# danini/multi-h

Measured on AMD Instinct MI355X. Metric: scored homography hypotheses/sec (50k pts x 100k models), higher is better.
Workload: dtype f64

## Files before the change

### multi-h_amd/csrc/dlt4.hip

```cpp

#include "mh_kernels.hpp"
#include "mh_device.hpp"
#include "mh_sampler.hpp"

namespace mh {


__device__ __forceinline__ void rr_pair(int r, int slot, int& p, int& q)
{
    const int k = slot + 1;
    const int a = (r + k) % 9, b = (r + 9 - k) % 9;
    p = a < b ? a : b;
    q = a < b ? b : a;
}

constexpr int HPW = 16;
constexpr int WROWS = 17, WCOLS = 9;

__device__ __forceinline__ void wave_sync()
{
#ifdef MH_DLT_WAVE_FENCES
    __builtin_amdgcn_fence(__ATOMIC_RELEASE, "wavefront");
    __builtin_amdgcn_wave_barrier();
    __builtin_amdgcn_fence(__ATOMIC_ACQUIRE, "wavefront");
#else
    asm volatile("" ::: "memory");
    __builtin_amdgcn_wave_barrier();
    asm volatile("" ::: "memory");
#endif
}

__device__ __forceinline__ void null9_sweeps(double (*W)[HPW], int hs, int slot, bool live)
{
#define WE(r, c) W[(r) * WCOLS + (c)][hs]
    for (int sweep = 0; sweep < 30; ++sweep) {
        int rotated = 0;
        for (int r = 0; r < 9; ++r) {
            int p, q;
            rr_pair(r, slot, p, q);
            double alpha = 0.0, beta = 0.0, gamma = 0.0;
#pragma unroll
            for (int i = 0; i < 8; ++i) {
                const double wp = WE(i, p), wq = WE(i, q);
                alpha = alpha + wp * wp;
                beta = beta + wq * wq;
                gamma = gamma + wp * wq;
            }
            const bool rot = live && (gamma != 0.0) && (gamma * gamma > 1e-30 * (alpha * beta)) &&
                             (alpha >= 1e-28) && (beta >= 1e-28);
            if (rot) {
                ++rotated;
                const double zeta = (beta - alpha) / (2.0 * gamma);
                const double sg = (zeta >= 0.0) ? 1.0 : -1.0;
                const double t = sg / (fabs(zeta) + sqrt(1.0 + zeta * zeta));
                const double c = 1.0 / sqrt(1.0 + t * t);
                const double s = c * t;
#pragma unroll
                for (int i = 0; i < WROWS; ++i) {
                    const double wp = WE(i, p), wq = WE(i, q);
                    WE(i, p) = c * wp - s * wq;
                    WE(i, q) = s * wp + c * wq;
                }
            }
            wave_sync();
        }
        if (!__any(rotated)) break;
    }
#undef WE
}

__device__ __forceinline__ void null9_vector(double (*W)[HPW], int hs, double g[9])
{
#define WE(r, c) W[(r) * WCOLS + (c)][hs]
    int jm = 0;
    double best = 0.0;
    for (int j = 0; j < 9; ++j) {
        double a = 0.0;
        for (int i = 0; i < 8; ++i) a = a + WE(i, j) * WE(i, j);
        if (j == 0 || a < best) { best = a; jm = j; }
    }
    for (int j = 0; j < 9; ++j) g[j] = WE(8 + j, jm);
#undef WE
}

template <int SAMPLER, class... TABLE>
__global__ void __launch_bounds__(256) __attribute__((amdgpu_num_vgpr(72)))
k_dlt4_lds(const double* __restrict__ x1, const double* __restrict__ y1,
       const double* __restrict__ x2, const double* __restrict__ y2, int N,
       unsigned long long seed, long long first, int M, int* __restrict__ idx_out,
       double* __restrict__ H_out, TABLE... table)
{
    static_assert(sizeof...(TABLE) == dlt_sampler_args(SAMPLER), "the local sampler takes nbr, k, uniform_per_16; the segment sampler cluster_begin, trials, first");
    __builtin_amdgcn_s_setprio(3);
    __shared__ double sW[4][WROWS * WCOLS][HPW];
    const int lane = threadIdx.x & 63;
    const int wave = threadIdx.x >> 6;
    const int hs = lane & (HPW - 1);
    const int slot = lane >> 4;
    const int m = (blockIdx.x * 4 + wave) * HPW + hs;
    const bool live = m < M;
    double (*W)[HPW] = sW[wave];
#define WE(r, c) W[(r) * WCOLS + (c)][hs]

    int id[4] = { 0, 0, 0, 0 };
    double sx[4], sy[4], dx[4], dy[4];
    if (live) sample4_by(seed, (unsigned long long)(first + m), (unsigned int)N, id, table...);
#pragma unroll
    for (int k = 0; k < 4; ++k) {
        sx[k] = x1[id[k]]; sy[k] = y1[id[k]]; dx[k] = x2[id[k]]; dy[k] = y2[id[k]];
    }
    if (live && slot == 0 && idx_out) {
#pragma unroll
        for (int k = 0; k < 4; ++k) idx_out[4 * (size_t)m + k] = id[k];
    }
    double cx1 = ((sx[0] + sx[1]) + sx[2]) + sx[3], cy1 = ((sy[0] + sy[1]) + sy[2]) + sy[3];
    double cx2 = ((dx[0] + dx[1]) + dx[2]) + dx[3], cy2 = ((dy[0] + dy[1]) + dy[2]) + dy[3];
    cx1 = cx1 * 0.25; cy1 = cy1 * 0.25; cx2 = cx2 * 0.25; cy2 = cy2 * 0.25;
    double d1 = 0.0, d2 = 0.0;
#pragma unroll
    for (int k = 0; k < 4; ++k) {
        const double ax = sx[k] - cx1, ay = sy[k] - cy1, bx = dx[k] - cx2, by = dy[k] - cy2;
        d1 = d1 + sqrt(ax * ax + ay * ay);
        d2 = d2 + sqrt(bx * bx + by * by);
    }
    const double s1 = sqrt(2.0) / (d1 * 0.25), s2 = sqrt(2.0) / (d2 * 0.25);

    {
        double x = 0.0, y = 0.0, u = 0.0, v = 0.0;
#pragma unroll
        for (int k = 0; k < 4; ++k)
            if (k == slot) {
                x = (sx[k] - cx1) * s1; y = (sy[k] - cy1) * s1;
                u = (dx[k] - cx2) * s2; v = (dy[k] - cy2) * s2;
            }
        const int r0 = 2 * slot, r1 = 2 * slot + 1;
        WE(r0, 0) = -x; WE(r0, 1) = -y; WE(r0, 2) = -1.0; WE(r0, 3) = 0.0; WE(r0, 4) = 0.0;
        WE(r0, 5) = 0.0; WE(r0, 6) = u * x; WE(r0, 7) = u * y; WE(r0, 8) = u;
        WE(r1, 0) = 0.0; WE(r1, 1) = 0.0; WE(r1, 2) = 0.0; WE(r1, 3) = -x; WE(r1, 4) = -y;
        WE(r1, 5) = -1.0; WE(r1, 6) = v * x; WE(r1, 7) = v * y; WE(r1, 8) = v;
        if (slot < 3)
            for (int i = 3 * slot; i < 3 * slot + 3; ++i)
                for (int j = 0; j < 9; ++j) WE(8 + i, j) = (i == j) ? 1.0 : 0.0;
    }
    __syncthreads();

    null9_sweeps(W, hs, slot, live);

    if (live && slot == 0) {
        double g[9];
        null9_vector(W, hs, g);
        double A1[9];
#pragma unroll
        for (int r = 0; r < 3; ++r) {
            const double a = g[3 * r], b = g[3 * r + 1], c = g[3 * r + 2];
            A1[3 * r] = a * s1;
            A1[3 * r + 1] = b * s1;
            A1[3 * r + 2] = (c - (a * s1) * cx1) - (b * s1) * cy1;
        }
        const double is2 = 1.0 / s2;
        double Hh[9];
#pragma unroll
        for (int j = 0; j < 3; ++j) {
            Hh[j] = A1[j] * is2 + cx2 * A1[6 + j];
            Hh[3 + j] = A1[3 + j] * is2 + cy2 * A1[6 + j];
            Hh[6 + j] = A1[6 + j];
        }
        double fro = 0.0;
#pragma unroll
        for (int j = 0; j < 9; ++j) fro = fro + Hh[j] * Hh[j];
        double sc = 1.0 / sqrt(fro);
        if (Hh[8] < 0.0) sc = -sc;
        double* out = H_out + 9 * (size_t)m;
#pragma unroll
        for (int j = 0; j < 9; ++j) out[j] = Hh[j] * sc;
    }
#undef WE
}

struct Col { double v[WROWS]; };

template <int CTRL, int BANK_MASK>
__device__ __forceinline__ double dpp_merge(double old, double src)
{
    const int lo = __builtin_amdgcn_update_dpp(__double2loint(old), __double2loint(src), CTRL, 0xF, BANK_MASK, false);
    const int hi = __builtin_amdgcn_update_dpp(__double2hiint(old), __double2hiint(src), CTRL, 0xF, BANK_MASK, false);
    return __hiloint2double(hi, lo);
}

__device__ __forceinline__ void shift_columns(Col& a, Col& b, Col& c)
{
#pragma unroll
    for (int i = 0; i < WROWS; ++i) {
        c.v[i] = dpp_merge<0x114 , 0xE>(c.v[i], b.v[i]);
        b.v[i] = dpp_merge<0x104 , 0x7>(b.v[i], a.v[i]);
    }
}

__device__ __forceinline__ int rotate_pair(Col& P, Col& Q, bool swapped, bool live)
{
    double alpha = 0.0, beta = 0.0, gamma = 0.0;
#pragma unroll
    for (int i = 0; i < 8; ++i) {
        const double wp = P.v[i], wq = Q.v[i];
        alpha = alpha + wp * wp;
        beta = beta + wq * wq;
        gamma = gamma + wp * wq;
    }
    const bool rot = live && (gamma != 0.0) && (gamma * gamma > 1e-30 * (alpha * beta)) &&
                     (alpha >= 1e-28) && (beta >= 1e-28);
    if (rot) {
        const double zeta = (beta - alpha) / (2.0 * gamma);
        const bool pos = swapped ? (zeta > 0.0) : (zeta >= 0.0);
        const double sg = pos ? 1.0 : -1.0;
        const double t = sg / (fabs(zeta) + sqrt(1.0 + zeta * zeta));
        const double c = 1.0 / sqrt(1.0 + t * t);
        const double s = c * t;
#pragma unroll
        for (int i = 0; i < WROWS; ++i) {
            const double wp = P.v[i], wq = Q.v[i];
            P.v[i] = c * wp - s * wq;
            Q.v[i] = s * wp + c * wq;
        }
    }
    return rot ? 1 : 0;
}

__host__ __device__ constexpr unsigned swapped_rounds(int s)
{
    unsigned m = 0;
    for (int r = 0; r < 9; ++r) {
        const int k = s + 1, a = (r + k) % 9, b = (r + 9 - k) % 9;
        if (a > b) m |= 1u << r;
    }
    return m;
}

__device__ __forceinline__ void dlt_column(int c, const double* x, const double* y, const double* u, const double* v, Col& out)
{
#pragma unroll
    for (int k = 0; k < 4; ++k) {
        const double e0[9] = { -x[k], -y[k], -1.0, 0.0, 0.0, 0.0, u[k] * x[k], u[k] * y[k], u[k] };
        const double e1[9] = { 0.0, 0.0, 0.0, -x[k], -y[k], -1.0, v[k] * x[k], v[k] * y[k], v[k] };
        double r0 = e0[0], r1 = e1[0];
#pragma unroll
        for (int j = 1; j < 9; ++j) {
            r0 = (c == j) ? e0[j] : r0;
            r1 = (c == j) ? e1[j] : r1;
        }
        out.v[2 * k] = r0;
        out.v[2 * k + 1] = r1;
    }
#pragma unroll
    for (int i = 0; i < 9; ++i) out.v[8 + i] = (i == c) ? 1.0 : 0.0;
}

__device__ __forceinline__ double column_norm(const Col& a)
{
    double n = 0.0;
#pragma unroll
    for (int i = 0; i < 8; ++i) n = n + a.v[i] * a.v[i];
    return n;
}

template <int SAMPLER, class... TABLE>
__global__ void __launch_bounds__(256)
k_dlt4(const double* __restrict__ x1, const double* __restrict__ y1,
       const double* __restrict__ x2, const double* __restrict__ y2, int N,
       unsigned long long seed, long long first, int M, int* __restrict__ idx_out,
       double* __restrict__ H_out, TABLE... table)
{
    static_assert(sizeof...(TABLE) == dlt_sampler_args(SAMPLER), "the local sampler takes nbr, k, uniform_per_16; the segment sampler cluster_begin, trials, first");
    __builtin_amdgcn_s_setprio(3);
    __shared__ double sN[4][9][HPW];
    __shared__ double sK[4][6][HPW];
    const int lane = threadIdx.x & 63;
    const int wave = threadIdx.x >> 6;
    const int slot = (lane >> 2) & 3;
    const int hs = (lane >> 4) * 4 + (lane & 3);
    const int m = (blockIdx.x * 4 + wave) * HPW + hs;
    const bool live = m < M;

    Col A, B, C;
    {
        int id[4] = { 0, 0, 0, 0 };
        double sx[4], sy[4], dx[4], dy[4];
        if (live) sample4_by(seed, (unsigned long long)(first + m), (unsigned int)N, id, table...);
#pragma unroll
        for (int k = 0; k < 4; ++k) {
            sx[k] = x1[id[k]]; sy[k] = y1[id[k]]; dx[k] = x2[id[k]]; dy[k] = y2[id[k]];
        }
        if (live && slot == 0 && idx_out) {
#pragma unroll
            for (int k = 0; k < 4; ++k) idx_out[4 * (size_t)m + k] = id[k];
        }
        double cx1 = ((sx[0] + sx[1]) + sx[2]) + sx[3], cy1 = ((sy[0] + sy[1]) + sy[2]) + sy[3];
        double cx2 = ((dx[0] + dx[1]) + dx[2]) + dx[3], cy2 = ((dy[0] + dy[1]) + dy[2]) + dy[3];
        cx1 = cx1 * 0.25; cy1 = cy1 * 0.25; cx2 = cx2 * 0.25; cy2 = cy2 * 0.25;
        double d1 = 0.0, d2 = 0.0;
#pragma unroll
        for (int k = 0; k < 4; ++k) {
            const double ax = sx[k] - cx1, ay = sy[k] - cy1, bx = dx[k] - cx2, by = dy[k] - cy2;
            d1 = d1 + sqrt(ax * ax + ay * ay);
            d2 = d2 + sqrt(bx * bx + by * by);
        }
        const double s1 = sqrt(2.0) / (d1 * 0.25), s2 = sqrt(2.0) / (d2 * 0.25);
        if (slot == 0) {
            sK[wave][0][hs] = s1; sK[wave][1][hs] = s2; sK[wave][2][hs] = cx1;
            sK[wave][3][hs] = cy1; sK[wave][4][hs] = cx2; sK[wave][5][hs] = cy2;
        }
        double x[4], y[4], u[4], v[4];
#pragma unroll
        for (int k = 0; k < 4; ++k) {
            x[k] = (sx[k] - cx1) * s1; y[k] = (sy[k] - cy1) * s1;
            u[k] = (dx[k] - cx2) * s2; v[k] = (dy[k] - cy2) * s2;
        }
        dlt_column(slot + 1, x, y, u, v, A);
        dlt_column(8 - slot, x, y, u, v, B);
        dlt_column(0, x, y, u, v, C);
    }

    const unsigned sw = slot == 0 ? swapped_rounds(0) : slot == 1 ? swapped_rounds(1) : slot == 2 ? swapped_rounds(2) : swapped_rounds(3);
    for (int sweep = 0; sweep < 30; ++sweep) {
        unsigned long long rotated = 0;
#pragma unroll 1
        for (int r = 0; r < 9; r += 3) {
            rotated |= __ballot(rotate_pair(A, B, (sw >> r) & 1u, live));
            shift_columns(A, B, C);
            rotated |= __ballot(rotate_pair(B, C, (sw >> (r + 1)) & 1u, live));
            shift_columns(B, C, A);
            rotated |= __ballot(rotate_pair(C, A, (sw >> (r + 2)) & 1u, live));
            shift_columns(C, A, B);
        }
        if (rotated == 0) break;
    }

    sN[wave][slot + 1][hs] = column_norm(A);
    sN[wave][8 - slot][hs] = column_norm(B);
    if (slot == 0) sN[wave][0][hs] = column_norm(C);
    wave_sync();
    int jm = 0;
    {
        double best = 0.0;
        for (int j = 0; j < 9; ++j) {
            const double a = sN[wave][j][hs];
            if (j == 0 || a < best) { best = a; jm = j; }
        }
    }
    wave_sync();
    if (jm == slot + 1) {
#pragma unroll
        for (int j = 0; j < 9; ++j) sN[wave][j][hs] = A.v[8 + j];
    } else if (jm == 8 - slot) {
#pragma unroll
        for (int j = 0; j < 9; ++j) sN[wave][j][hs] = B.v[8 + j];
    } else if (jm == 0 && slot == 0) {
#pragma unroll
        for (int j = 0; j < 9; ++j) sN[wave][j][hs] = C.v[8 + j];
    }
    wave_sync();

    if (live && slot == 0) {
        double g[9];
#pragma unroll
        for (int j = 0; j < 9; ++j) g[j] = sN[wave][j][hs];
        const double s1 = sK[wave][0][hs], s2 = sK[wave][1][hs], cx1 = sK[wave][2][hs];
        const double cy1 = sK[wave][3][hs], cx2 = sK[wave][4][hs], cy2 = sK[wave][5][hs];
        double A1[9];
#pragma unroll
        for (int r = 0; r < 3; ++r) {
            const double a = g[3 * r], b = g[3 * r + 1], c = g[3 * r + 2];
            A1[3 * r] = a * s1;
            A1[3 * r + 1] = b * s1;
            A1[3 * r + 2] = (c - (a * s1) * cx1) - (b * s1) * cy1;
        }
        const double is2 = 1.0 / s2;
        double Hh[9];
#pragma unroll
        for (int j = 0; j < 3; ++j) {
            Hh[j] = A1[j] * is2 + cx2 * A1[6 + j];
            Hh[3 + j] = A1[3 + j] * is2 + cy2 * A1[6 + j];
            Hh[6 + j] = A1[6 + j];
        }
        double fro = 0.0;
#pragma unroll
        for (int j = 0; j < 9; ++j) fro = fro + Hh[j] * Hh[j];
        double sc = 1.0 / sqrt(fro);
        if (Hh[8] < 0.0) sc = -sc;
        double* out = H_out + 9 * (size_t)m;
#pragma unroll
        for (int j = 0; j < 9; ++j) out[j] = Hh[j] * sc;
    }
}

__global__ void __launch_bounds__(256)
k_fund8(const double* __restrict__ x1, const double* __restrict__ y1,
        const double* __restrict__ x2, const double* __restrict__ y2, int N,
        unsigned long long seed, long long first, int M, int* __restrict__ idx_out,
        double* __restrict__ F_out)
{
    __shared__ double sW[4][WROWS * WCOLS][HPW];
    const int lane = threadIdx.x & 63;
    const int wave = threadIdx.x >> 6;
    const int hs = lane & (HPW - 1);
    const int slot = lane >> 4;
    const int m = (blockIdx.x * 4 + wave) * HPW + hs;
    const bool live = m < M;
    double (*W)[HPW] = sW[wave];
#define WE(r, c) W[(r) * WCOLS + (c)][hs]

    int id[8] = { 0, 0, 0, 0, 0, 0, 0, 0 };
    if (live) sample_tuple<8, 256>(seed, (unsigned long long)(first + m), (unsigned int)N, id);
    double sx[8], sy[8], dx[8], dy[8];
#pragma unroll
    for (int k = 0; k < 8; ++k) { sx[k] = x1[id[k]]; sy[k] = y1[id[k]]; dx[k] = x2[id[k]]; dy[k] = y2[id[k]]; }
    if (live && slot == 0 && idx_out) {
#pragma unroll
        for (int k = 0; k < 8; ++k) idx_out[8 * (size_t)m + k] = id[k];
    }
    double cx1 = sx[0], cy1 = sy[0], cx2 = dx[0], cy2 = dy[0];
#pragma unroll
    for (int k = 1; k < 8; ++k) { cx1 = cx1 + sx[k]; cy1 = cy1 + sy[k]; cx2 = cx2 + dx[k]; cy2 = cy2 + dy[k]; }
    cx1 = cx1 * 0.125; cy1 = cy1 * 0.125; cx2 = cx2 * 0.125; cy2 = cy2 * 0.125;
    double d1 = 0.0, d2 = 0.0;
#pragma unroll
    for (int k = 0; k < 8; ++k) {
        const double ax = sx[k] - cx1, ay = sy[k] - cy1, bx = dx[k] - cx2, by = dy[k] - cy2;
        d1 = d1 + sqrt(ax * ax + ay * ay);
        d2 = d2 + sqrt(bx * bx + by * by);
    }
    const double s1 = sqrt(2.0) / (d1 * 0.125), s2 = sqrt(2.0) / (d2 * 0.125);

#pragma unroll
    for (int k = 0; k < 8; ++k)
        if ((k >> 1) == slot) {
            const double x = (sx[k] - cx1) * s1, y = (sy[k] - cy1) * s1;
            const double u = (dx[k] - cx2) * s2, v = (dy[k] - cy2) * s2;
            WE(k, 0) = u * x; WE(k, 1) = u * y; WE(k, 2) = u;
            WE(k, 3) = v * x; WE(k, 4) = v * y; WE(k, 5) = v;
            WE(k, 6) = x; WE(k, 7) = y; WE(k, 8) = 1.0;
        }
    if (slot < 3)
        for (int i = 3 * slot; i < 3 * slot + 3; ++i)
            for (int j = 0; j < 9; ++j) WE(8 + i, j) = (i == j) ? 1.0 : 0.0;
    __syncthreads();

    null9_sweeps(W, hs, slot, live);

    if (live && slot == 0) {
        double g[9];
        null9_vector(W, hs, g);
        double Mm[9], V[9], D[3];
        for (int i = 0; i < 3; ++i)
            for (int j = 0; j < 3; ++j) {
                double a = 0.0;
                for (int k = 0; k < 3; ++k) a = a + g[3 * k + i] * g[3 * k + j];
                Mm[3 * i + j] = a;
            }
        jacobi_sym_dev(3, Mm, V, D);
        int jm = 0;
        for (int j = 1; j < 3; ++j) if (D[j] < D[jm]) jm = j;
        const double v0 = V[0 * 3 + jm], v1 = V[1 * 3 + jm], v2 = V[2 * 3 + jm];
        double Fn[9];
        for (int r = 0; r < 3; ++r) {
            const double w = (g[3 * r] * v0 + g[3 * r + 1] * v1) + g[3 * r + 2] * v2;
            Fn[3 * r] = g[3 * r] - w * v0;
            Fn[3 * r + 1] = g[3 * r + 1] - w * v1;
            Fn[3 * r + 2] = g[3 * r + 2] - w * v2;
        }
        double B[9];
        for (int r = 0; r < 3; ++r) {
            const double a = Fn[3 * r] * s1, b = Fn[3 * r + 1] * s1;
            B[3 * r] = a; B[3 * r + 1] = b;
            B[3 * r + 2] = (Fn[3 * r + 2] - a * cx1) - b * cy1;
        }
        double Fh[9];
        const double tx = s2 * cx2, ty = s2 * cy2;
        for (int j = 0; j < 3; ++j) {
            Fh[j] = s2 * B[j];
            Fh[3 + j] = s2 * B[3 + j];
            Fh[6 + j] = (B[6 + j] - tx * B[j]) - ty * B[3 + j];
        }
        double fro = 0.0;
        for (int j = 0; j < 9; ++j) fro = fro + Fh[j] * Fh[j];
        double sc = 1.0 / sqrt(fro);
        if (Fh[8] < 0.0) sc = -sc;
        double* out = F_out + 9 * (size_t)m;
        for (int j = 0; j < 9; ++j) out[j] = Fh[j] * sc;
    }
#undef WE
}

__device__ __forceinline__ double det3_rows(const double* r0, const double* r1, const double* r2)
{
    return (r0[0] * (r1[1] * r2[2] - r1[2] * r2[1]) - r0[1] * (r1[0] * r2[2] - r1[2] * r2[0])) +
           r0[2] * (r1[0] * r2[1] - r1[1] * r2[0]);
}

__device__ __forceinline__ double cubic_newton(double c0, double c1, double c2, double c3, double t)
{
    double p = ((c3 * t + c2) * t + c1) * t + c0;
    for (int it = 0; it < 4; ++it) {
        const double dp = (3.0 * c3 * t + 2.0 * c2) * t + c1;
        const double tn = t - p / dp;
        const double pn = ((c3 * tn + c2) * tn + c1) * tn + c0;
        if (!(fabs(pn) <= fabs(p)) || !(fabs(tn) < 1e300)) break;
        t = tn; p = pn;
    }
    return t;
}

struct CubicRoots { double t0, t1, t2; int n; };

__device__ __forceinline__ CubicRoots cubic_real_roots(double c0, double c1, double c2, double c3)
{
    const double qnan = __longlong_as_double(0x7ff8000000000000ll);
    const double a = c2 / c3, b = c1 / c3, c = c0 / c3;
    const double Q = (a * a - 3.0 * b) / 9.0;
    const double R = ((2.0 * a * a * a - 9.0 * a * b) + 27.0 * c) / 54.0;
    const double Q3 = Q * Q * Q;
    const double disc = R * R - Q3;
    const double a3 = a / 3.0;
    const bool usable = (fabs(a) < 1e300) && (fabs(b) < 1e300) && (fabs(c) < 1e300) && (fabs(disc) < 1e300);
    const bool three = disc < 0.0;
    const double theta = acos(R / sqrt(Q3));
    const double sq = -2.0 * sqrt(Q);
    const double two_pi = 6.283185307179586476925286766559;
    const double u0 = sq * cos(theta / 3.0) - a3;
    const double u1 = sq * cos((theta + two_pi) / 3.0) - a3;
    const double u2 = sq * cos((theta - two_pi) / 3.0) - a3;
    double A = cbrt(fabs(R) + sqrt(disc));
    if (R >= 0.0) A = -A;
    const double B = (A == 0.0) ? 0.0 : Q / A;
    const double w0 = (A + B) - a3;
    const double w1 = -0.5 * (A + B) - a3;
    const int nr = !usable ? 0 : three ? 3 : (disc == 0.0 && Q > 0.0) ? 2 : 1;
    double r0 = nr == 0 ? qnan : cubic_newton(c0, c1, c2, c3, three ? u0 : w0);
    double r1 = nr < 2 ? qnan : cubic_newton(c0, c1, c2, c3, three ? u1 : w1);
    double r2 = nr < 3 ? qnan : cubic_newton(c0, c1, c2, c3, u2);
    { const bool sw = (r1 < r0) || (r0 != r0 && r1 == r1); const double lo = sw ? r1 : r0, hi = sw ? r0 : r1; r0 = lo; r1 = hi; }
    { const bool sw = (r2 < r1) || (r1 != r1 && r2 == r2); const double lo = sw ? r2 : r1, hi = sw ? r1 : r2; r1 = lo; r2 = hi; }
    { const bool sw = (r1 < r0) || (r0 != r0 && r1 == r1); const double lo = sw ? r1 : r0, hi = sw ? r0 : r1; r0 = lo; r1 = hi; }
    return CubicRoots{ r0, r1, r2, nr };
}

__global__ void __launch_bounds__(256)
k_fund7(const double* __restrict__ x1, const double* __restrict__ y1,
        const double* __restrict__ x2, const double* __restrict__ y2, int N,
        unsigned long long seed, long long first, int M, int* __restrict__ idx_out,
        double* __restrict__ F_out, int* __restrict__ nvalid_out)
{
    __shared__ double sW[4][WROWS * WCOLS][HPW];
    const int lane = threadIdx.x & 63;
    const int wave = threadIdx.x >> 6;
    const int hs = lane & (HPW - 1);
    const int slot = lane >> 4;
    const int m = (blockIdx.x * 4 + wave) * HPW + hs;
    const bool live = m < M;
    double (*W)[HPW] = sW[wave];
#define WE(r, c) W[(r) * WCOLS + (c)][hs]

    int id[7] = { 0, 0, 0, 0, 0, 0, 0 };
    if (live) sample_tuple<7, 256>(seed, (unsigned long long)(first + m), (unsigned int)N, id);
    double sx[7], sy[7], dx[7], dy[7];
#pragma unroll
    for (int k = 0; k < 7; ++k) { sx[k] = x1[id[k]]; sy[k] = y1[id[k]]; dx[k] = x2[id[k]]; dy[k] = y2[id[k]]; }
    if (live && slot == 0 && idx_out) {
#pragma unroll
        for (int k = 0; k < 7; ++k) idx_out[7 * (size_t)m + k] = id[k];
    }
    double cx1 = sx[0], cy1 = sy[0], cx2 = dx[0], cy2 = dy[0];
#pragma unroll
    for (int k = 1; k < 7; ++k) { cx1 = cx1 + sx[k]; cy1 = cy1 + sy[k]; cx2 = cx2 + dx[k]; cy2 = cy2 + dy[k]; }
    cx1 = cx1 / 7.0; cy1 = cy1 / 7.0; cx2 = cx2 / 7.0; cy2 = cy2 / 7.0;
    double d1 = 0.0, d2 = 0.0;
#pragma unroll
    for (int k = 0; k < 7; ++k) {
        const double ax = sx[k] - cx1, ay = sy[k] - cy1, bx = dx[k] - cx2, by = dy[k] - cy2;
        d1 = d1 + sqrt(ax * ax + ay * ay);
        d2 = d2 + sqrt(bx * bx + by * by);
    }
    const double s1 = sqrt(2.0) / (d1 / 7.0), s2 = sqrt(2.0) / (d2 / 7.0);

#pragma unroll
    for (int k = 0; k < 7; ++k)
        if ((k >> 1) == slot) {
            const double x = (sx[k] - cx1) * s1, y = (sy[k] - cy1) * s1;
            const double u = (dx[k] - cx2) * s2, v = (dy[k] - cy2) * s2;
            WE(k, 0) = u * x; WE(k, 1) = u * y; WE(k, 2) = u;
            WE(k, 3) = v * x; WE(k, 4) = v * y; WE(k, 5) = v;
            WE(k, 6) = x; WE(k, 7) = y; WE(k, 8) = 1.0;
        }
    if (slot == 3)
        for (int j = 0; j < 9; ++j) WE(7, j) = 0.0;
    if (slot < 3)
        for (int i = 3 * slot; i < 3 * slot + 3; ++i)
            for (int j = 0; j < 9; ++j) WE(8 + i, j) = (i == j) ? 1.0 : 0.0;
    __syncthreads();

    null9_sweeps(W, hs, slot, live);

    int j2 = 0, j1 = -1;
    {
        double best2 = 0.0, best1 = 0.0;
        for (int j = 0; j < 9; ++j) {
            double a = 0.0;
            for (int i = 0; i < 8; ++i) a = a + WE(i, j) * WE(i, j);
            if (j == 0 || a < best2) { best2 = a; j2 = j; }
        }
        for (int j = 0; j < 9; ++j) {
            if (j == j2) continue;
            double a = 0.0;
            for (int i = 0; i < 8; ++i) a = a + WE(i, j) * WE(i, j);
            if (j1 < 0 || a < best1) { best1 = a; j1 = j; }
        }
    }
    double G2[9], D[9];
#pragma unroll
    for (int j = 0; j < 9; ++j) { G2[j] = WE(8 + j, j2); D[j] = WE(8 + j, j1) - G2[j]; }
    const double c0 = det3_rows(G2, G2 + 3, G2 + 6);
    const double c3 = det3_rows(D, D + 3, D + 6);
    const double c1 = (det3_rows(D, G2 + 3, G2 + 6) + det3_rows(G2, D + 3, G2 + 6)) + det3_rows(G2, G2 + 3, D + 6);
    const double c2 = (det3_rows(G2, D + 3, D + 6) + det3_rows(D, G2 + 3, D + 6)) + det3_rows(D, D + 3, G2 + 6);
    const CubicRoots roots = cubic_real_roots(c0, c1, c2, c3);
    const int nroots = roots.n;

    const double t = slot == 0 ? roots.t0 : slot == 1 ? roots.t1 : roots.t2;
    double Fo[9];
    bool ok = live && slot < nroots;
    {
        double B[9];
#pragma unroll
        for (int r = 0; r < 3; ++r) {
            const double f0 = G2[3 * r] + t * D[3 * r], f1 = G2[3 * r + 1] + t * D[3 * r + 1], f2 = G2[3 * r + 2] + t * D[3 * r + 2];
            const double a = f0 * s1, b = f1 * s1;
            B[3 * r] = a; B[3 * r + 1] = b;
            B[3 * r + 2] = (f2 - a * cx1) - b * cy1;
        }
        double Fh[9];
        const double tx = s2 * cx2, ty = s2 * cy2;
#pragma unroll
        for (int j = 0; j < 3; ++j) {
            Fh[j] = s2 * B[j];
            Fh[3 + j] = s2 * B[3 + j];
            Fh[6 + j] = (B[6 + j] - tx * B[j]) - ty * B[3 + j];
        }
        double fro = 0.0;
#pragma unroll
        for (int j = 0; j < 9; ++j) fro = fro + Fh[j] * Fh[j];
        double sc = 1.0 / sqrt(fro);
        if (Fh[8] < 0.0) sc = -sc;
#pragma unroll
        for (int j = 0; j < 9; ++j) {
            Fo[j] = Fh[j] * sc;
            ok = ok && (fabs(Fo[j]) < 1e300);
        }
    }
    const unsigned long long okb = __ballot(ok);
    const int ok0 = (int)((okb >> hs) & 1ull), ok1 = (int)((okb >> (HPW + hs)) & 1ull), ok2 = (int)((okb >> (2 * HPW + hs)) & 1ull);
    const int nv = ok0 + ok1 + ok2;
    if (live && slot < 3) {
        const int place = slot == 0 ? 0 : slot == 1 ? ok0 : ok0 + ok1;
        if (ok) {
            double* out = F_out + (3 * (size_t)m + place) * 9;
#pragma unroll
            for (int j = 0; j < 9; ++j) out[j] = Fo[j];
        }
        if (slot >= nv) {
            const double qnan = __longlong_as_double(0x7ff8000000000000ll);
            double* out = F_out + (3 * (size_t)m + slot) * 9;
#pragma unroll
            for (int j = 0; j < 9; ++j) out[j] = qnan;
        }
        if (slot == 0 && nvalid_out) nvalid_out[m] = nv;
    }
#undef WE
}

hipError_t launch_fund7(const Points& p, unsigned long long seed, long long first, int M,
                        int* idx_out, double* F_out, int* nvalid_out, hipStream_t s)
{
    if (M <= 0) return hipSuccess;
    const int per_block = 4 * HPW;
    hipLaunchKernelGGL(k_fund7, dim3((M + per_block - 1) / per_block), dim3(256), 0, s, p.x1, p.y1,
                       p.x2, p.y2, p.n, seed, first, M, idx_out, F_out, nvalid_out);
    return hipGetLastError();
}

hipError_t launch_fund8(const Points& p, unsigned long long seed, long long first, int M,
                        int* idx_out, double* F_out, hipStream_t s)
{
    if (M <= 0) return hipSuccess;
    const int per_block = 4 * HPW;
    hipLaunchKernelGGL(k_fund8, dim3((M + per_block - 1) / per_block), dim3(256), 0, s, p.x1, p.y1,
                       p.x2, p.y2, p.n, seed, first, M, idx_out, F_out);
    return hipGetLastError();
}

hipError_t launch_dlt4(const Points& p, unsigned long long seed, long long first, int M,
                       int* idx_out, double* H_out, hipStream_t s, int variant, Dlt4Local local)
{
    if (M <= 0) return hipSuccess;
    const int per_block = 4 * HPW;
    const dim3 grid((M + per_block - 1) / per_block);
    if (local.nbr) {
        if (local.k < 1 || local.k >= p.n || local.uniform_per_16 < 0 || local.uniform_per_16 > 16) return hipErrorInvalidValue;
        if (variant == 1)
            hipLaunchKernelGGL((k_dlt4_lds<DLT_SAMPLER_LOCAL, const int*, int, int>), grid, dim3(256), 0, s, p.x1, p.y1,
                               p.x2, p.y2, p.n, seed, first, M, idx_out, H_out, local.nbr, local.k, local.uniform_per_16);
        else
            hipLaunchKernelGGL((k_dlt4<DLT_SAMPLER_LOCAL, const int*, int, int>), grid, dim3(256), 0, s, p.x1, p.y1,
                               p.x2, p.y2, p.n, seed, first, M, idx_out, H_out, local.nbr, local.k, local.uniform_per_16);
    } else if (variant == 1)
        hipLaunchKernelGGL(k_dlt4_lds<DLT_SAMPLER_UNIFORM>, grid, dim3(256), 0, s, p.x1, p.y1,
                           p.x2, p.y2, p.n, seed, first, M, idx_out, H_out);
    else
        hipLaunchKernelGGL(k_dlt4<DLT_SAMPLER_UNIFORM>, grid, dim3(256), 0, s, p.x1, p.y1,
                           p.x2, p.y2, p.n, seed, first, M, idx_out, H_out);
    return hipGetLastError();
}

hipError_t launch_dlt4_segments(const double* x1, const double* y1, const double* x2, const double* y2, int total, const int* begin,
                                int trials, unsigned long long seed, long long first, int M, int* idx_out, double* H_out,
                                hipStream_t s)
{
    if (M <= 0) return hipSuccess;
    if (total < 4 || trials < 1 || !begin || !idx_out || !H_out) return hipErrorInvalidValue;
    const int per_block = 4 * HPW;
    hipLaunchKernelGGL((k_dlt4<DLT_SAMPLER_SEGMENT, const int*, int, long long>), dim3((M + per_block - 1) / per_block), dim3(256), 0,
                       s, x1, y1, x2, y2, total, seed, first, M, idx_out, H_out, begin, trials, first);
    return hipGetLastError();
}

}
```

Before: 13.86 million.

## Hand one column per Jacobi round and split point loads across lane banks

Replaces the two-column DPP shift after each one-sided Jacobi rotation with a single-column hand-over. A new bank-role schedule, checked at compile time, keeps the circle ordering intact while moving one column per round. Convergence now stops after nine consecutive clean rounds instead of checking once per full sweep, and the loop body is unrolled to six rounds. Each lane in a bank now loads only one of the four points and builds the centroid and scale with DPP reductions, so lanes no longer load all four points. The trade-off is more complex index bookkeeping to find which register holds which column at the end.

```diff
diff --git a/multi-h_amd/csrc/dlt4.hip b/multi-h_amd/csrc/dlt4.hip
--- a/multi-h_amd/csrc/dlt4.hip
+++ b/multi-h_amd/csrc/dlt4.hip
@@ -187,13 +187,70 @@
     return __hiloint2double(hi, lo);
 }
 
-__device__ __forceinline__ void shift_columns(Col& a, Col& b, Col& c)
-{
-#pragma unroll
-    for (int i = 0; i < WROWS; ++i) {
-        c.v[i] = dpp_merge<0x114 , 0xE>(c.v[i], b.v[i]);
-        b.v[i] = dpp_merge<0x104 , 0x7>(b.v[i], a.v[i]);
-    }
+constexpr int DLT_ROUND_CAP = 30 * 9;
+constexpr int DLT_LAYOUT_PERIOD = 18;
+
+__host__ __device__ constexpr int bank_role(int bank, int t)
+{
+    return (((t & 1) ? 0x1243 : 0x2134) >> (4 * bank)) & 0xF;
+}
+__host__ __device__ constexpr int column_p(int bank, int t)
+{
+    const int k = bank_role(bank, t);
+    return (t % 9 + ((k & 1) ? k : 9 - k)) % 9;
+}
+__host__ __device__ constexpr int column_q(int bank, int t)
+{
+    const int k = bank_role(bank, t);
+    return (t % 9 + ((k & 1) ? 9 - k : k)) % 9;
+}
+__host__ __device__ constexpr unsigned swapped_rounds(int bank)
+{
+    unsigned m = 0;
+    for (int t = 0; t < DLT_LAYOUT_PERIOD; ++t)
+        if (column_p(bank, t) > column_q(bank, t)) m |= 1u << t;
+    return m;
+}
+__host__ __device__ constexpr bool layout_follows_schedule()
+{
+    int col[4][3] = {};
+    for (int b = 0; b < 4; ++b) {
+        col[b][0] = column_p(b, 0);
+        col[b][1] = column_q(b, 0);
+        col[b][2] = bank_role(b, 0) == 2 ? 0 : -1;
+    }
+    for (int t = 0; t < 2 * DLT_LAYOUT_PERIOD; ++t) {
+        const int P = t % 3, Q = (t + 1) % 3, S = (t + 2) % 3, r = t % 9;
+        unsigned seen = 0;
+        for (int b = 0; b < 4; ++b) {
+            const int k = bank_role(b, t);
+            if (col[b][P] != column_p(b, t) || col[b][Q] != column_q(b, t)) return false;
+            const int x = (r + k) % 9, y = (r + 9 - k) % 9;
+            const int p = x < y ? x : y, q = x < y ? y : x;
+            const int lo = col[b][P] < col[b][Q] ? col[b][P] : col[b][Q], hi = col[b][P] < col[b][Q] ? col[b][Q] : col[b][P];
+            if (lo != p || hi != q) return false;
+            if (k == 2 && col[b][S] != r) return false;
+            seen |= 1u << k;
+        }
+        if (seen != 0x1Eu) return false;
+        int got[4] = {};
+        for (int b = 0; b < 4; ++b) got[b] = (t & 1) ? col[(b + 1) & 3][P] : col[(b + 3) & 3][P];
+        for (int b = 0; b < 4; ++b)
+            if (bank_role(b, t) != 2) col[b][S] = got[b];
+    }
+    return true;
+}
+static_assert(layout_follows_schedule(), "the one-column hand-over does not reproduce the circle schedule");
+static_assert(bank_role(3, 0) == 2 && bank_role(2, 1) == 2, "hand_on's bank masks spare the bank of pair 2");
+static_assert(DLT_ROUND_CAP % 6 == 0 && DLT_LAYOUT_PERIOD % 6 == 0, "the loop body is six rounds");
+
+template <bool ODD>
+__device__ __forceinline__ void hand_on(Col& s, const Col& p)
+{
+#pragma unroll
+    for (int i = 0; i < WROWS; ++i)
+        s.v[i] = ODD ? dpp_merge<0x12C , 0xB>(s.v[i], p.v[i])
+                     : dpp_merge<0x124 , 0x7>(s.v[i], p.v[i]);
 }
 
 __device__ __forceinline__ int rotate_pair(Col& P, Col& Q, bool swapped, bool live)
@@ -218,40 +275,30 @@
 #pragma unroll
         for (int i = 0; i < WROWS; ++i) {
             const double wp = P.v[i], wq = Q.v[i];
-            P.v[i] = c * wp - s * wq;
-            Q.v[i] = s * wp + c * wq;
+            const double sp = s * wp, cq = c * wq, cp = c * wp, sq = s * wq;
+            P.v[i] = cp - sq;
+            Q.v[i] = sp + cq;
         }
     }
     return rot ? 1 : 0;
 }
 
-__host__ __device__ constexpr unsigned swapped_rounds(int s)
-{
-    unsigned m = 0;
-    for (int r = 0; r < 9; ++r) {
-        const int k = s + 1, a = (r + k) % 9, b = (r + 9 - k) % 9;
-        if (a > b) m |= 1u << r;
-    }
-    return m;
-}
-
-__device__ __forceinline__ void dlt_column(int c, const double* x, const double* y, const double* u, const double* v, Col& out)
-{
-#pragma unroll
-    for (int k = 0; k < 4; ++k) {
-        const double e0[9] = { -x[k], -y[k], -1.0, 0.0, 0.0, 0.0, u[k] * x[k], u[k] * y[k], u[k] };
-        const double e1[9] = { 0.0, 0.0, 0.0, -x[k], -y[k], -1.0, v[k] * x[k], v[k] * y[k], v[k] };
-        double r0 = e0[0], r1 = e1[0];
-#pragma unroll
-        for (int j = 1; j < 9; ++j) {
-            r0 = (c == j) ? e0[j] : r0;
-            r1 = (c == j) ? e1[j] : r1;
-        }
-        out.v[2 * k] = r0;
-        out.v[2 * k + 1] = r1;
-    }
-#pragma unroll
-    for (int i = 0; i < 9; ++i) out.v[8 + i] = (i == c) ? 1.0 : 0.0;
+__device__ __forceinline__ double sum_over_banks(double v)
+{
+    double acc = dpp_merge<0x124, 0xF>(v, v) + v;
+    acc = dpp_merge<0x124, 0xF>(acc, acc) + v;
+    acc = dpp_merge<0x124, 0xF>(acc, acc) + v;
+    double out = acc;
+    out = dpp_merge<0x124, 0x1>(out, acc);
+    out = dpp_merge<0x128, 0x2>(out, acc);
+    out = dpp_merge<0x12C, 0x4>(out, acc);
+    return out;
+}
+template <int B, int K>
+__device__ __forceinline__ double from_bank(double old, double src)
+{
+    constexpr int d = (B - K + 4) & 3;
+    return dpp_merge<(d == 0 ? 0xE4  : 0x120 + 4 * d ), 1 << B>(old, src);
 }
 
 __device__ __forceinline__ double column_norm(const Col& a)
@@ -275,7 +322,7 @@
     __shared__ double sK[4][6][HPW];
     const int lane = threadIdx.x & 63;
     const int wave = threadIdx.x >> 6;
-    const int slot = (lane >> 2) & 3;
+    const int bank = (lane >> 2) & 3;
     const int hs = (lane >> 4) * 4 + (lane & 3);
     const int m = (blockIdx.x * 4 + wave) * HPW + hs;
     const bool live = m < M;
@@ -283,60 +330,77 @@
     Col A, B, C;
     {
         int id[4] = { 0, 0, 0, 0 };
-        double sx[4], sy[4], dx[4], dy[4];
         if (live) sample4_by(seed, (unsigned long long)(first + m), (unsigned int)N, id, table...);
-#pragma unroll
-        for (int k = 0; k < 4; ++k) {
-            sx[k] = x1[id[k]]; sy[k] = y1[id[k]]; dx[k] = x2[id[k]]; dy[k] = y2[id[k]];
-        }
-        if (live && slot == 0 && idx_out) {
+        if (live && bank == 0 && idx_out) {
 #pragma unroll
             for (int k = 0; k < 4; ++k) idx_out[4 * (size_t)m + k] = id[k];
         }
-        double cx1 = ((sx[0] + sx[1]) + sx[2]) + sx[3], cy1 = ((sy[0] + sy[1]) + sy[2]) + sy[3];
-        double cx2 = ((dx[0] + dx[1]) + dx[2]) + dx[3], cy2 = ((dy[0] + dy[1]) + dy[2]) + dy[3];
-        cx1 = cx1 * 0.25; cy1 = cy1 * 0.25; cx2 = cx2 * 0.25; cy2 = cy2 * 0.25;
-        double d1 = 0.0, d2 = 0.0;
-#pragma unroll
-        for (int k = 0; k < 4; ++k) {
-            const double ax = sx[k] - cx1, ay = sy[k] - cy1, bx = dx[k] - cx2, by = dy[k] - cy2;
-            d1 = d1 + sqrt(ax * ax + ay * ay);
-            d2 = d2 + sqrt(bx * bx + by * by);
-        }
+        const int mine = bank == 0 ? id[0] : bank == 1 ? id[1] : bank == 2 ? id[2] : id[3];
+        const double sx = x1[mine], sy = y1[mine], dx = x2[mine], dy = y2[mine];
+        const double cx1 = sum_over_banks(sx) * 0.25, cy1 = sum_over_banks(sy) * 0.25;
+        const double cx2 = sum_over_banks(dx) * 0.25, cy2 = sum_over_banks(dy) * 0.25;
+        const double ax = sx - cx1, ay = sy - cy1, bx = dx - cx2, by = dy - cy2;
+        const double d1 = sum_over_banks(0.0 + sqrt(ax * ax + ay * ay));
+        const double d2 = sum_over_banks(0.0 + sqrt(bx * bx + by * by));
         const double s1 = sqrt(2.0) / (d1 * 0.25), s2 = sqrt(2.0) / (d2 * 0.25);
-        if (slot == 0) {
+        if (bank == 0) {
             sK[wave][0][hs] = s1; sK[wave][1][hs] = s2; sK[wave][2][hs] = cx1;
             sK[wave][3][hs] = cy1; sK[wave][4][hs] = cx2; sK[wave][5][hs] = cy2;
         }
-        double x[4], y[4], u[4], v[4];
-#pragma unroll
-        for (int k = 0; k < 4; ++k) {
-            x[k] = (sx[k] - cx1) * s1; y[k] = (sy[k] - cy1) * s1;
-            u[k] = (dx[k] - cx2) * s2; v[k] = (dy[k] - cy2) * s2;
-        }
-        dlt_column(slot + 1, x, y, u, v, A);
-        dlt_column(8 - slot, x, y, u, v, B);
-        dlt_column(0, x, y, u, v, C);
-    }
-
-    const unsigned sw = slot == 0 ? swapped_rounds(0) : slot == 1 ? swapped_rounds(1) : slot == 2 ? swapped_rounds(2) : swapped_rounds(3);
-    for (int sweep = 0; sweep < 30; ++sweep) {
-        unsigned long long rotated = 0;
+        const double x = ax * s1, y = ay * s1, u = bx * s2, v = by * s2;
+        const double nx = -x, ny = -y, ux = u * x, uy = u * y, vx = v * x, vy = v * y;
+        static_assert(column_p(0, 0) == 5 && column_q(0, 0) == 4 && column_p(1, 0) == 3 && column_q(1, 0) == 6 &&
+                      column_p(2, 0) == 1 && column_q(2, 0) == 8 && column_p(3, 0) == 7 && column_q(3, 0) == 2, "the table above");
+        const double p_odd = bank == 0 ? -1.0 : 0.0, q_even = bank == 3 ? -1.0 : 0.0;
+#define MH_ROWS(k)                                                                                                           \
+        A.v[2 * k] = from_bank<3, k>(from_bank<2, k>(0.0, ny), uy);                                                          \
+        A.v[2 * k + 1] = from_bank<3, k>(from_bank<1, k>(p_odd, nx), vy);                                                    \
+        B.v[2 * k] = from_bank<2, k>(from_bank<1, k>(q_even, ux), u);                                                        \
+        B.v[2 * k + 1] = from_bank<2, k>(from_bank<1, k>(from_bank<0, k>(0.0, ny), vx), v);                                  \
+        C.v[2 * k] = from_bank<3, k>(0.0, nx);                                                                               \
+        C.v[2 * k + 1] = 0.0;
+        MH_ROWS(0) MH_ROWS(1) MH_ROWS(2) MH_ROWS(3)
+#undef MH_ROWS
+        const int cp = bank == 0 ? 5 : bank == 1 ? 3 : bank == 2 ? 1 : 7;
+        const int cq = bank == 0 ? 4 : bank == 1 ? 6 : bank == 2 ? 8 : 2;
+#pragma unroll
+        for (int i = 0; i < 9; ++i) {
+            A.v[8 + i] = (i == cp) ? 1.0 : 0.0;
+            B.v[8 + i] = (i == cq) ? 1.0 : 0.0;
+            C.v[8 + i] = (i == 0) ? 1.0 : 0.0;
+        }
+    }
+
+    const unsigned sw = bank == 0 ? swapped_rounds(0) : bank == 1 ? swapped_rounds(1) : bank == 2 ? swapped_rounds(2) : swapped_rounds(3);
+    int t = 0;
+    {
+        int clean = 0, phase = 0;
+#define MH_ROUND(P, Q, S, I)                                                                                                 \
+        if (clean < 9) {                                                                                                     \
+            const bool any = __ballot(rotate_pair(P, Q, (sw >> (phase + I)) & 1u, live)) != 0;                               \
+            hand_on<(I & 1) != 0>(S, P);                                                                                     \
+            ++t;                                                                                                             \
+            clean = any ? 0 : clean + 1;                                                                                     \
+        }
 #pragma unroll 1
-        for (int r = 0; r < 9; r += 3) {
-            rotated |= __ballot(rotate_pair(A, B, (sw >> r) & 1u, live));
-            shift_columns(A, B, C);
-            rotated |= __ballot(rotate_pair(B, C, (sw >> (r + 1)) & 1u, live));
-            shift_columns(B, C, A);
-            rotated |= __ballot(rotate_pair(C, A, (sw >> (r + 2)) & 1u, live));
-            shift_columns(C, A, B);
-        }
-        if (rotated == 0) break;
-    }
-
-    sN[wave][slot + 1][hs] = column_norm(A);
-    sN[wave][8 - slot][hs] = column_norm(B);
-    if (slot == 0) sN[wave][0][hs] = column_norm(C);
+        while (t < DLT_ROUND_CAP && clean < 9) {
+            MH_ROUND(A, B, C, 0)
+            MH_ROUND(B, C, A, 1)
+            MH_ROUND(C, A, B, 2)
+            MH_ROUND(A, B, C, 3)
+            MH_ROUND(B, C, A, 4)
+            MH_ROUND(C, A, B, 5)
+            phase = phase == DLT_LAYOUT_PERIOD - 6 ? 0 : phase + 6;
+        }
+#undef MH_ROUND
+    }
+
+    const int r = t % 9, rp = t % 3;
+    const int role = bank_role(bank, t), colP = column_p(bank, t), colQ = column_q(bank, t);
+    const double nA = column_norm(A), nB = column_norm(B), nC = column_norm(C);
+    sN[wave][colP][hs] = rp == 0 ? nA : rp == 1 ? nB : nC;
+    sN[wave][colQ][hs] = rp == 0 ? nB : rp == 1 ? nC : nA;
+    if (role == 2) sN[wave][r][hs] = rp == 0 ? nC : rp == 1 ? nA : nB;
     wave_sync();
     int jm = 0;
     {
@@ -347,19 +411,17 @@
         }
     }
     wave_sync();
-    if (jm == slot + 1) {
-#pragma unroll
-        for (int j = 0; j < 9; ++j) sN[wave][j][hs] = A.v[8 + j];
-    } else if (jm == 8 - slot) {
-#pragma unroll
-        for (int j = 0; j < 9; ++j) sN[wave][j][hs] = B.v[8 + j];
-    } else if (jm == 0 && slot == 0) {
-#pragma unroll
-        for (int j = 0; j < 9; ++j) sN[wave][j][hs] = C.v[8 + j];
+    {
+        const int held = jm == colP ? rp : jm == colQ ? rp + 1 : (role == 2 && jm == r) ? rp + 2 : -1;
+        const int set = held >= 3 ? held - 3 : held;
+        if (set >= 0) {
+#pragma unroll
+            for (int j = 0; j < 9; ++j) sN[wave][j][hs] = set == 0 ? A.v[8 + j] : set == 1 ? B.v[8 + j] : C.v[8 + j];
+        }
     }
     wave_sync();
 
-    if (live && slot == 0) {
+    if (live && bank == 0) {
         double g[9];
 #pragma unroll
         for (int j = 0; j < 9; ++j) g[j] = sN[wave][j][hs];
@@ -367,11 +429,11 @@
         const double cy1 = sK[wave][3][hs], cx2 = sK[wave][4][hs], cy2 = sK[wave][5][hs];
         double A1[9];
 #pragma unroll
-        for (int r = 0; r < 3; ++r) {
-            const double a = g[3 * r], b = g[3 * r + 1], c = g[3 * r + 2];
-            A1[3 * r] = a * s1;
-            A1[3 * r + 1] = b * s1;
-            A1[3 * r + 2] = (c - (a * s1) * cx1) - (b * s1) * cy1;
+        for (int r3 = 0; r3 < 3; ++r3) {
+            const double a = g[3 * r3], b = g[3 * r3 + 1], c = g[3 * r3 + 2];
+            A1[3 * r3] = a * s1;
+            A1[3 * r3 + 1] = b * s1;
+            A1[3 * r3 + 2] = (c - (a * s1) * cx1) - (b * s1) * cy1;
         }
         const double is2 = 1.0 / s2;
         double Hh[9];
```

Result: no change. 13.93 million (median of 6 runs) (+0.5%).
